# jimouris/draft-mouris-cfrg-mastic

Hardware: AMD Instinct MI355X
Metric: VIDPF report x prefix evals/sec at 1/2/4/8 GPUs; % of int-VALU peak (higher is better)
Workload: dtype u32

## Files before the change

draft-mouris-cfrg-mastic_amd/csrc/keccak.hpp:

```cpp
#pragma once
#include "common.hpp"

#define KECCAK_RATE 168
#define KECCAK_RATE_WORDS 42

struct KState {
    u32x2 a[25];
};

#define KR(x, y) KECCAK_ROTC[(x) + 5 * (y)]
static constexpr int KECCAK_ROTC[25] = {0,  1,  62, 28, 27, 36, 44, 6,  55, 20, 3,  10, 43,
                                        25, 39, 41, 45, 15, 21, 8,  18, 2,  61, 56, 14};

MH_D u32x2 chi1(u32x2 a, u32x2 b, u32x2 c) {
    return u32x2{(uint32_t)__builtin_amdgcn_bitop3_b32(a.lo, b.lo, c.lo, 0xD2),
                 (uint32_t)__builtin_amdgcn_bitop3_b32(a.hi, b.hi, c.hi, 0xD2)};
}

template <int U = 12, bool FUSE_D = true>
MH_D void keccak_p12(KState& s) {
    static constexpr uint32_t RCL[12] = {0x8000808bu, 0x0000008bu, 0x00008089u, 0x00008003u,
                                         0x00008002u, 0x00000080u, 0x0000800au, 0x8000000au,
                                         0x80008081u, 0x00008080u, 0x80000001u, 0x80008008u};
    static constexpr uint32_t RCH[12] = {0x00000000u, 0x80000000u, 0x80000000u, 0x80000000u,
                                         0x80000000u, 0x80000000u, 0x00000000u, 0x80000000u,
                                         0x80000000u, 0x80000000u, 0x00000000u, 0x80000000u};
    u32x2* A = s.a;
#pragma unroll U
    for (int round = 0; round < 12; round++) {
        u32x2 C[5], D[5];
#pragma unroll
        for (int x = 0; x < 5; x++) {
            u32x2 t = xor3_64(A[x], A[x + 5], A[x + 10]);
            C[x] = xor3_64(t, A[x + 15], A[x + 20]);
        }
        u32x2 B[25];
        if constexpr (FUSE_D) {
#pragma unroll
            for (int x = 0; x < 5; x++) D[x] = rotl64(C[(x + 1) % 5], 1);
#pragma unroll
            for (int x = 0; x < 5; x++)
#pragma unroll
                for (int y = 0; y < 5; y++)
                    B[y + 5 * ((2 * x + 3 * y) % 5)] = rotl64(xor3_64(A[x + 5 * y], C[(x + 4) % 5], D[x]), KR(x, y));
        } else {
#pragma unroll
            for (int x = 0; x < 5; x++) D[x] = xor64(C[(x + 4) % 5], rotl64(C[(x + 1) % 5], 1));
#pragma unroll
            for (int x = 0; x < 5; x++)
#pragma unroll
                for (int y = 0; y < 5; y++)
                    B[y + 5 * ((2 * x + 3 * y) % 5)] = rotl64(xor64(A[x + 5 * y], D[x]), KR(x, y));
        }
#pragma unroll
        for (int y = 0; y < 5; y++)
#pragma unroll
            for (int x = 0; x < 5; x++)
                A[x + 5 * y] = chi1(B[x + 5 * y], B[(x + 1) % 5 + 5 * y], B[(x + 2) % 5 + 5 * y]);
        A[0].lo ^= RCL[round];
        A[0].hi ^= RCH[round];
    }
}

struct KHalf {
    uint32_t a[25];
};

MH_D uint32_t pair_swap(uint32_t v) {
    return (uint32_t)__builtin_amdgcn_mov_dpp((int)v, 0xB1, 0xF, 0xF, false);
}

MH_D uint32_t pair_rotl(uint32_t v, int r) {
    if (r == 0) return v;
    const uint32_t p = pair_swap(v);
    return r < 32 ? __builtin_amdgcn_alignbit(v, p, 32 - r) : __builtin_amdgcn_alignbit(p, v, 64 - r);
}

template <int U = 12>
MH_D void keccak_p12_pair(KHalf& s, bool hi) {
    static constexpr uint32_t RCL[12] = {0x8000808bu, 0x0000008bu, 0x00008089u, 0x00008003u,
                                         0x00008002u, 0x00000080u, 0x0000800au, 0x8000000au,
                                         0x80008081u, 0x00008080u, 0x80000001u, 0x80008008u};
    static constexpr uint32_t RCH[12] = {0x00000000u, 0x80000000u, 0x80000000u, 0x80000000u,
                                         0x80000000u, 0x80000000u, 0x00000000u, 0x80000000u,
                                         0x80000000u, 0x80000000u, 0x00000000u, 0x80000000u};
    uint32_t* A = s.a;
#pragma unroll U
    for (int round = 0; round < 12; round++) {
        uint32_t C[5], D[5];
#pragma unroll
        for (int x = 0; x < 5; x++) C[x] = xor3_u32(xor3_u32(A[x], A[x + 5], A[x + 10]), A[x + 15], A[x + 20]);
#pragma unroll
        for (int x = 0; x < 5; x++) D[x] = pair_rotl(C[(x + 1) % 5], 1);
        uint32_t B[25];
#pragma unroll
        for (int x = 0; x < 5; x++)
#pragma unroll
            for (int y = 0; y < 5; y++)
                B[y + 5 * ((2 * x + 3 * y) % 5)] = pair_rotl(xor3_u32(A[x + 5 * y], C[(x + 4) % 5], D[x]), KR(x, y));
#pragma unroll
        for (int y = 0; y < 5; y++)
#pragma unroll
            for (int x = 0; x < 5; x++)
                A[x + 5 * y] = (uint32_t)__builtin_amdgcn_bitop3_b32(B[x + 5 * y], B[(x + 1) % 5 + 5 * y],
                                                                    B[(x + 2) % 5 + 5 * y], 0xD2);
        A[0] ^= hi ? RCH[round] : RCL[round];
    }
}

MH_D uint32_t kword(const KState& s, int j) {
    return (j & 1) ? s.a[j >> 1].hi : s.a[j >> 1].lo;
}
MH_D void kxor_word(KState& s, int j, uint32_t v) {
    if (j & 1) s.a[j >> 1].hi ^= v; else s.a[j >> 1].lo ^= v;
}

template <class Loader>
MH_D int sponge_absorb_words(KState& s, int f, int nbytes, Loader ld) {
    if (nbytes <= 0) return f;
    const int q = f >> 2;
    const int sh = f & 3;
    const int off = sh ? 1 : 0;
    const int amt = (32 - 8 * sh) & 31;
    const int nw = (nbytes + 3) >> 2;
    const int end = f + nbytes;
    for (int b = 0;; b++) {
        const int base = KECCAK_RATE_WORDS * b - q - off;
        uint32_t w[KECCAK_RATE_WORDS + 1];
#pragma unroll
        for (int j = 0; j < KECCAK_RATE_WORDS + 1; j++) {
            const int m = base + j;
            w[j] = ld(m < 0 ? 0 : (m >= nw ? nw - 1 : m));
        }
#pragma unroll
        for (int j = 0; j < KECCAK_RATE_WORDS + 1; j++) {
            const int m = base + j;
            w[j] = (m >= 0 && m < nw) ? w[j] : 0u;
        }
#pragma unroll
        for (int j = 0; j < KECCAK_RATE_WORDS; j++) kxor_word(s, j, __builtin_amdgcn_alignbit(w[j + 1], w[j], amt));
        if (end >= KECCAK_RATE * (b + 1)) {
            keccak_p12(s);
            if (end == KECCAK_RATE * (b + 1)) return 0;
        } else {
            return end - KECCAK_RATE * b;
        }
    }
}

MH_D void sponge_pad(KState& s, int f, uint32_t domain) {
    const int q = f >> 2;
    const uint32_t dw = domain << (8 * (f & 3));
// ... 58 lines not shown
```

draft-mouris-cfrg-mastic_amd/csrc/kernels.hpp:

```cpp
#pragma once
#include "aes.hpp"
#include "flp.hpp"
#include "keccak.hpp"

enum PfxId {
    PFX_EXT = 0,
    PFX_CONV,
    PFX_NODE,
    PFX_ONEHOT,
    PFX_PAYLOAD,
    PFX_EVAL,
    PFX_QUERY,
    PFX_PROOF_SHARE,
    PFX_JR_PART,
    PFX_JR_SEED,
    PFX_JR,
    PFX_PROVE_RAND,
    PFX_TREE,
    PFX_COUNT
};

struct PrefixState {
    KState st;
    int f;
// ... 533 lines not shown
        } else {
            const uint32_t* const sd2[2] = {cv, cv};
            const uint32_t cvv[2] = {c0, c1};
            uint32_t* const ov[2] = {o[0], o[1]};
            fixed_key_block_n<2>(TL, rkc, sd2, cvv, ov);
        }
        bool sus = false;
        const int e0 = EPB * b;
#pragma unroll
        for (int k = 0; k < 2 * EPB; k++) {
            const int e = e0 + k;
            const uint32_t top = EPB == 2 ? o[k >> 1][2 * (k & 1) + 1] : o[k][3];
            if (e < e_hi && (k < EPB || two)) sus |= top == ~0u;
        }
        if (__builtin_expect(__any(sus), 0) || b == force_slow_blk || b + 1 == force_slow_blk) break;
        __builtin_amdgcn_s_waitcnt(0x0F70);
#pragma unroll
        for (int k = 0; k < 2 * EPB; k++) {
            const int e = e0 + k;
            if (e < e_hi && (k < EPB || two)) {
                E x = F::from_words(&o[k / EPB][(k % EPB) * F::W32]);
                if (t) x = F::add(x, cwv[k]);
                pl_store<F>(out, row0 + e, S, r, x);
            }
        }
        e_fast = min(e_hi, e0 + 2 * EPB);
    }
    if (e_fast < e_hi) {
        typename EvalStream<F, false>::type st;
        st.init(cv);
        for (int e = 0; e < e_hi; e++) {
            asm volatile("" ::: "memory");
            const E x = st.next(TL, rkc);
            if (e >= e_fast) put(e, x);
        }
    }
}

#define EVAL_WAVES 16
#ifndef MASTIC_EMIT_WAIT
#define MASTIC_EMIT_WAIT 1
#endif
#ifndef MASTIC_CTR_GROUPS
#define MASTIC_CTR_GROUPS 1
#endif
#define EVAL_PROOF_WAVES 8
#ifndef EVAL_MIN_WAVES
#define EVAL_MIN_WAVES 5
#endif
#ifndef EVAL_FC_MIN_WAVES
#define EVAL_FC_MIN_WAVES 4
#endif
#define EVAL_VGPR_ATTR __attribute__((amdgpu_waves_per_eu(FC ? EVAL_FC_MIN_WAVES : EVAL_MIN_WAVES)))
#define EVAL_SYNC_WORDS 40
#define EVAL_LDS_BYTES (AES_PERM_LDS_WORDS * 4 + 2 * 64 * 11 * 16 + 4 * EVAL_SYNC_WORDS)
template <class F, bool GEN, bool FC, bool SPLIT = false>
__global__ __launch_bounds__(64 * EVAL_WAVES) EVAL_VGPR_ATTR
void k_eval_aes(McParams p, Planes pl, AesArgs a) {
    typedef typename F::E E;
    extern __shared__ uint4 eval_lds[];
    uint32_t* T = (uint32_t*)eval_lds;
    uint4* RKE = eval_lds + AES_PERM_LDS_WORDS / 4;
    uint4* RKC = RKE + 64 * 11;
    uint32_t* next_parent = (uint32_t*)(RKC + 64 * 11);
    uint32_t* next_proof = next_parent + 1;
    uint32_t* parent_done = next_parent + 8;
    if ((uint32_t)(uintptr_t)(const __attribute__((address_space(3))) uint4*)eval_lds != 0u) __builtin_trap();

    const int S = pl.stride;
    const int S_in = FC ? a.in_stride : S;
    const int lane = threadIdx.x & 63;
    const int wave = __builtin_amdgcn_readfirstlane(threadIdx.x >> 6);
    const int r = blockIdx.x * 64 + lane;
    const uint32_t lb = (uint32_t)r * 4u;
    {
        uint32_t* ke = (uint32_t*)RKE;
        uint32_t* kc = (uint32_t*)RKC;
        constexpr int KR = (44 + EVAL_WAVES - 1) / EVAL_WAVES;
        uint32_t xe[KR], xc[KR];
#pragma unroll
        for (int j = 0; j < KR; j++) {
            const int i = wave + j * EVAL_WAVES;
            if (i < 44) {
                xe[j] = pld(pl.rk_ext + (size_t)i * S, lb);
                xc[j] = pld(pl.rk_conv + (size_t)i * S, lb);
            }
        }
        aes_perm_fill(T, threadIdx.x, 64 * EVAL_WAVES);
#pragma unroll
        for (int j = 0; j < KR; j++) {
            const int i = wave + j * EVAL_WAVES;
            if (i < 44) {
                ke[lane * 44 + i] = aes_perm_key_word(i, xe[j]);
                kc[lane * 44 + i] = aes_perm_key_word(i, xc[j]);
            }
        }
    }
    if (threadIdx.x < EVAL_SYNC_WORDS) next_parent[threadIdx.x] = (SPLIT && threadIdx.x >= 8) ? ~0u : 0u;
    __syncthreads();
    const int aes_waves = a.aes_waves;
    if (wave >= aes_waves && a.pv_nodes > 0 && !(a.dbg_skip & 1)) {
        if (a.proof_prio == 1) __builtin_amdgcn_s_setprio(1);
        if (a.proof_prio == 2) __builtin_amdgcn_s_setprio(2);
        const int nbeg = (blockIdx.y * (EVAL_WAVES - aes_waves) + (wave - aes_waves)) * a.pv_npw;
        const int nend = min(nbeg + a.pv_npw, a.pv_nodes);
        const int pl_ = a.pv_level;
        uint32_t* ohg = a.pv_onehot + (size_t)blockIdx.x * a.oh_gstride;
        const uint32_t lt = (uint32_t)lane * 4u;
        uint32_t pcw[8];
#pragma unroll
        for (int j = 0; j < 8; j++) pcw[j] = pld(pl.cw_proof + ((size_t)pl_ * 8 + j) * S, lb);
        for (int node = nbeg; node < nend; node++) {
            uint32_t sd[4];
#pragma unroll
            for (int i = 0; i < 4; i++) sd[i] = pld(a.cs_in + ((size_t)node * 5 + i) * S_in, lb);
            const uint32_t t = pld(a.cs_in + ((size_t)node * 5 + 4) * S_in, lb);
            node_proof_one<FC>(a.np, a.np_f, p.bits, pl_, a.pv_path_bytes, sd, a.pv_child_path + node * 8, t, pcw,
                           [&](int j, uint32_t w) { pst(ohg + ((size_t)node * 8 + j) * a.bin_rstride, lt, w); });
        }
        if (a.proof_prio) __builtin_amdgcn_s_setprio(0);
    }
    const int wp0 = blockIdx.y * a.par_waves * a.ppw;
    const int wp1 = min(wp0 + a.par_waves * a.ppw, SPLIT ? a.n_parents * a.split : a.n_parents);
    const int pn_beg = 2 * wp0, pn_end = 2 * wp1;
    const bool fuse_ovl = FC && a.fuse_proofs == 1;
    auto parent_marked = [&](int q) -> bool {
        const uint32_t w = __hip_atomic_load(parent_done + (q >> 5), __ATOMIC_ACQUIRE, __HIP_MEMORY_SCOPE_WORKGROUP);
        return (__builtin_amdgcn_readfirstlane(w) >> (q & 31)) & 1u;
    };
    auto claim_node = [&]() -> int {
        uint32_t o = 0;
        if (lane == 0) o = atomicAdd(next_proof, 1u);
        return pn_beg + (int)__builtin_amdgcn_readfirstlane(o);
    };
    auto node_proof_at = [&](int node) {
        if (a.dbg_skip & 2) return;
        if (fuse_ovl)
            while (!parent_marked((node - pn_beg) >> 1)) __builtin_amdgcn_s_sleep(2);
        const int l = a.level;
        uint32_t* ohg = a.cur_onehot + (size_t)blockIdx.x * a.oh_gstride;
        const uint32_t lt = (uint32_t)lane * 4u;
        uint32_t pcw[8];
#pragma unroll
        for (int j = 0; j < 8; j++) pcw[j] = pld(pl.cw_proof + ((size_t)l * 8 + j) * S, lb);
        uint32_t sd[4];
#pragma unroll
        for (int i = 0; i < 4; i++) sd[i] = pld(a.cs_out + ((size_t)node * 5 + i) * S, lb);
        const uint32_t t = pld(a.cs_out + ((size_t)node * 5 + 4) * S, lb);
        node_proof_one<FC>(a.np, a.np_f, p.bits, l, a.cur_path_bytes, sd, a.cur_child_path + node * 8, t, pcw,
                       [&](int j, uint32_t w) { pst(ohg + ((size_t)node * 8 + j) * a.bin_rstride, lt, w); });
    };
    if (a.dbg_skip & 2) goto aes_done;
    if (fuse_ovl && wave >= aes_waves) goto aes_done;
    {
    if (a.aes_prio == 1) __builtin_amdgcn_s_setprio(1);
    if (a.aes_prio == 2) __builtin_amdgcn_s_setprio(2);
    const int l = a.level;
    const int vl = p.value_len;
    const int wl = vl * F::W32;
    const AesPerm TL{T, 4u * (uint32_t)(lane & 31), 128u + 4u * (uint32_t)(lane & 31)};
    const RkLds rke{RKE + lane * 11};
    const RkLds rkc{RKC + lane * 11};

    uint32_t scw[4];
#pragma unroll
    for (int i = 0; i < 4; i++) scw[i] = pld(pl.cw_seed + ((size_t)l * 4 + i) * S, lb);
    const uint32_t ccw = pld(pl.cw_ctrl + (size_t)l * S, lb);
    const uint32_t* wcw = pl.cw_w + (size_t)l * wl * S;

    const int K = SPLIT ? a.split : 1;
    constexpr int npass = SPLIT ? 2 : 1;
// ... 225 lines not shown
                if constexpr (EPB == 2)
                    sus = (o0[1] == ~0u) | (o1[1] == ~0u) | (two & ((o0[3] == ~0u) | (o1[3] == ~0u)));
                else
                    sus = (o0[3] == ~0u) | (o1[3] == ~0u);
                if (__builtin_expect(__any(sus), 0) || b == a.force_slow_blk) {
                    if (K > 1) {
                        if (lane == 0) atomicMin(split_first + (pi - pb), (uint32_t)e);
                        deferred = true;
                    }
                    break;
                }
#if MASTIC_EMIT_WAIT
                __builtin_amdgcn_s_waitcnt(0x0F70);
#endif
                emit(e, F::from_words(o0), F::from_words(o1), cwa, wpa);
                if constexpr (EPB == 2) {
                    if (two) emit(e + 1, F::from_words(o0 + 2), F::from_words(o1 + 2), cwb, wpb);
                }
                e_fast = e + 1 + (two ? 1 : 0);
            }
        }
        if (e_fast < e_hi && !deferred) {
            typename EvalStream<F, false>::type st0, st1;
            st0.init(cs0);
            st1.init(cs1);
            constexpr int G = EvalStream<F, false>::type::GROUP;
            for (int e0 = 0; e0 < e_hi; e0 += G) {
                asm volatile("" ::: "memory");
                st0.refill(st1, e_hi - e0, TL, rkc);
#pragma unroll
                for (int i = 0; i < G; i++) {
                    const int e = e0 + i;
                    if (e >= e_hi) break;
                    const E x0 = st0.next(TL, rkc);
                    const E x1 = st1.next(TL, rkc);
                    if (e >= e_fast) emit(e, x0, x1, load_cw(e), load_wp(e));
                }
            }
        }
        item = nxt;
    }
    }
    }
aes_done:
    if constexpr (FC) {
        if (a.fuse_proofs) {
            if (!fuse_ovl) __syncthreads();
#pragma unroll 1
            for (int node = claim_node(); node < pn_end; node = claim_node()) node_proof_at(node);
        }
    }
}

struct ProofArgs {
    int oh_gstride;
    int bin_rstride;
    int level;
    int n_nodes;
    int npw;
    int path_bytes;
    const uint32_t* child_path;
    const uint32_t* cs;
    uint32_t* onehot;
    const PrefixState* np;
    int f;
};

__global__ __launch_bounds__(256) void k_node_proof(McParams p, Planes pl, ProofArgs a) {
    const int S = pl.stride;
    const int lane = threadIdx.x & 63;
    const int wave = __builtin_amdgcn_readfirstlane(threadIdx.x >> 6);
    const int r = blockIdx.x * 64 + lane;
    const uint32_t lb = (uint32_t)r * 4u;
    const int nbeg = (blockIdx.y * 4 + wave) * a.npw;
    if (nbeg >= a.n_nodes) return;
    const int nend = min(nbeg + a.npw, a.n_nodes);
    const int l = a.level;
    uint32_t* ohg = a.onehot + (size_t)blockIdx.x * a.oh_gstride;
    const uint32_t lt = (uint32_t)lane * 4u;
    uint32_t pcw[8];
#pragma unroll
    for (int j = 0; j < 8; j++) pcw[j] = pld(pl.cw_proof + ((size_t)l * 8 + j) * S, lb);
    for (int node = nbeg; node < nend; node++) {
        uint32_t seed[4];
#pragma unroll
        for (int i = 0; i < 4; i++) seed[i] = pld(a.cs + ((size_t)node * 5 + i) * S, lb);
        const uint32_t t = pld(a.cs + ((size_t)node * 5 + 4) * S, lb);
        node_proof_one(a.np, a.f, p.bits, l, a.path_bytes, seed, a.child_path + node * 8, t, pcw,
                       [&](int j, uint32_t w) { pst(ohg + ((size_t)node * 8 + j) * a.bin_rstride, lt, w); });
    }
}

struct AbsorbArgs {
    const uint32_t* seg[2];
    int gstride[2];
    int rstride;
    int nbytes[2];
    int f[2];
    int prio;
    int dbg;
    int which0;
};
MH_D void absorb_setprio(int prio) {
    switch (prio) {
        case 0: break;
        case 1: __builtin_amdgcn_s_setprio(1); break;
// ... 27 lines not shown
    const int end = f + nb;
    auto load_block = [&](int b, uint32_t* w) {
        const int base = KECCAK_RATE_WORDS * b - q - off;
        if (base >= 0 && base + KECCAK_RATE_WORDS < nw) {
            const __amdgpu_buffer_rsrc_t rs = mh_rsrc(seg + (size_t)base * a.rstride);
            uint32_t so = 0;
#pragma unroll
            for (int j = 0; j < KECCAK_RATE_WORDS + 1; j++) {
                w[j] = pld_so(rs, lt, so);
                so += rowb;
                asm volatile("" : "+s"(so));
            }
        } else {
#pragma unroll
            for (int j = 0; j < KECCAK_RATE_WORDS + 1; j++) {
                const int m = base + j;
                const int mc = m < 0 ? 0 : (m >= nw ? nw - 1 : m);
                w[j] = pld(seg + (size_t)mc * a.rstride, lt);
            }
#pragma unroll
            for (int j = 0; j < KECCAK_RATE_WORDS + 1; j++) {
                const int m = base + j;
                w[j] = (m >= 0 && m < nw) ? w[j] : 0u;
            }
        }
    };
    uint32_t cur[KECCAK_RATE_WORDS + 1];
    load_block(0, cur);
    for (int b = 0;; b++) {
        const bool full = end >= KECCAK_RATE * (b + 1);
        const bool more = end > KECCAK_RATE * (b + 1);
#pragma unroll
        for (int j = 0; j < KECCAK_RATE_WORDS; j++) kxor_word(s, j, __builtin_amdgcn_alignbit(cur[j + 1], cur[j], amt));
        if (!full) break;
        asm volatile("" ::: "memory");
        if (more) load_block(b + 1, cur);
#ifdef MASTIC_EXPERIMENT_KNOBS
        if (a.dbg == 3)
            keccak_p12<2>(s);
        else
#endif
            keccak_p12(s);
        if (!more) break;
    }
#pragma unroll
    for (int i = 0; i < 25; i++) {
        pst(sp + (size_t)(2 * i) * S, lb, s.a[i].lo);
        pst(sp + (size_t)(2 * i + 1) * S, lb, s.a[i].hi);
    }
}

#ifndef ABSORB_MIN_WAVES
#define ABSORB_MIN_WAVES 5
#endif
__global__ __launch_bounds__(256) __attribute__((amdgpu_waves_per_eu(ABSORB_MIN_WAVES)))
void k_absorb_pair(Planes pl, AbsorbArgs a) {
    absorb_setprio(a.prio);
    const int h = threadIdx.x & 1;
    const int r = blockIdx.x * (int)(blockDim.x >> 1) + (int)(threadIdx.x >> 1);
    const int which = a.which0 + (int)blockIdx.y;
    if (r >= pl.stride) return;
    const int nb = a.nbytes[which];
    if (nb == 0) return;
    const int S = pl.stride;
    uint32_t* sp = which == 0 ? pl.sp_onehot : pl.sp_payload;
    const uint32_t* seg = a.seg[which] + (size_t)(r >> 6) * a.gstride[which];
    const uint32_t lbh = ((uint32_t)h * (uint32_t)S + (uint32_t)r) * 4u;
    const uint32_t lt = (uint32_t)(r & 63) * 4u;
    const uint32_t rowb = (uint32_t)a.rstride * 4u;
    const uint32_t lth = lt + (uint32_t)h * rowb;
    const uint32_t rowb2 = 2u * rowb;
    KHalf s;
#pragma unroll
    for (int i = 0; i < 25; i++) s.a[i] = pld(sp + (size_t)(2 * i) * S, lbh);
    const int f = a.f[which];
    const int q = f >> 2;
    const int sh = f & 3;
    const int off = sh ? 1 : 0;
    const int amt = (32 - 8 * sh) & 31;
    const int nw = (nb + 3) >> 2;
    const int end = f + nb;
    constexpr int NL = KECCAK_RATE_WORDS / 2 + 1;
    auto load_block = [&](int b, uint32_t* w) {
        const int base = KECCAK_RATE_WORDS * b - q - off;
        if (base >= 0 && base + KECCAK_RATE_WORDS + 1 < nw) {
            const __amdgpu_buffer_rsrc_t rs = mh_rsrc(seg + (size_t)base * a.rstride);
            uint32_t so = 0;
#pragma unroll
            for (int k = 0; k < NL; k++) {
                w[k] = pld_so(rs, lth, so);
                so += rowb2;
                asm volatile("" : "+s"(so));
            }
        } else {
#pragma unroll
            for (int k = 0; k < NL; k++) {
                const int m = base + 2 * k + h;
                const int mc = m < 0 ? 0 : (m >= nw ? nw - 1 : m);
                w[k] = pld(seg, (uint32_t)mc * rowb + lt);
            }
#pragma unroll
            for (int k = 0; k < NL; k++) {
                const int m = base + 2 * k + h;
                w[k] = (m >= 0 && m < nw) ? w[k] : 0u;
            }
        }
    };
    uint32_t cur[NL];
    if (a.dbg == 1 || a.dbg == 4) {
#pragma unroll
        for (int k = 0; k < NL; k++) cur[k] = lt + k;
    } else {
        load_block(0, cur);
    }
    for (int b = 0;; b++) {
        const bool full = end >= KECCAK_RATE * (b + 1);
        const bool more = end > KECCAK_RATE * (b + 1);
#pragma unroll
        for (int i = 0; i < 21; i++) {
            uint32_t nxt = 0u;
            if (sh) {
                const uint32_t x0 = pair_swap(cur[i]), x1 = pair_swap(cur[i + 1]);
                nxt = h ? x1 : x0;
            }
            s.a[i] ^= __builtin_amdgcn_alignbit(nxt, cur[i], amt);
        }
        if (!full) break;
        asm volatile("" ::: "memory");
        if (more && a.dbg != 1 && a.dbg != 4) load_block(b + 1, cur);
        if (a.dbg == 0 || a.dbg == 1) keccak_p12_pair(s, h != 0);
        else if (a.dbg == 4) __builtin_amdgcn_s_sleep(72);
        if (!more) break;
    }
#pragma unroll
    for (int i = 0; i < 25; i++) pst(sp + (size_t)(2 * i) * S, lbh, s.a[i]);
}

struct FinalArgs {
    int agg_id;
    int f_onehot;
    int f_payload;
};

template <class F>
__global__ __launch_bounds__(256) void k_finalize(McParams p, Planes pl, FinalArgs a, const PrefixState* pfx) {
    __shared__ uint32_t V[24 * 256];
    const int r = blockIdx.x * 256 + threadIdx.x;
    if (r >= pl.stride) return;
    const int S = pl.stride;
    uint32_t oh[8], pc[8];
    {
        KState s;
#pragma unroll
        for (int i = 0; i < 25; i++) s.a[i] = u32x2{pl.sp_onehot[(2 * i) * S + r], pl.sp_onehot[(2 * i + 1) * S + r]};
        sponge_pad(s, a.f_onehot, 0x01);
#pragma unroll
        for (int j = 0; j < 8; j++) oh[j] = kword(s, j);
#pragma unroll
        for (int i = 0; i < 25; i++) s.a[i] = u32x2{pl.sp_payload[(2 * i) * S + r], pl.sp_payload[(2 * i + 1) * S + r]};
        sponge_pad(s, a.f_payload, 0x01);
#pragma unroll
        for (int j = 0; j < 8; j++) pc[j] = kword(s, j);
    }
    typename F::E cnt = F::add(pl_load<F>(pl.rootsum, 0, S, r), F::from_u64((uint64_t)a.agg_id));
    const int t = threadIdx.x;
    for (int j = 0; j < 8; j++) V[j * 256 + t] = oh[j];
    for (int j = 0; j < F::W32; j++) V[(8 + j) * 256 + t] = F::word(cnt, j);
    for (int j = 0; j < 8; j++) V[(8 + F::W32 + j) * 256 + t] = pc[j];
    KState s;
    int f;
    load_prefix(pfx, PFX_EVAL, s, f);
    f = sponge_absorb_words(s, f, 64 + F::ENC, [&](int m) { return V[m * 256 + t]; });
    sponge_pad(s, f, 0x01);
#pragma unroll
    for (int j = 0; j < 8; j++) pl.eval_proof[j * S + r] = kword(s, j);
}

template <class F, class Put>
MH_D void squeeze_elems(KState& s, int count, Put put) {
    sponge_squeeze_vec<F::W32>(
        s, count, [&](const uint32_t* w) { return F::valid(F::from_words(w)); },
        [&](int e, const uint32_t* w) { put(e, F::from_words(w)); });
}
// ... 234 lines not shown
```

draft-mouris-cfrg-mastic_amd/csrc/mastic_hip.hip:

```cpp
#include "mastic_hip.h"

#include <dlfcn.h>
#include <rccl/rccl.h>

#include <algorithm>
#include <atomic>
#include <chrono>
#include <condition_variable>
#include <cstdarg>
#include <cstdio>
#include <cstring>
#include <map>
#include <memory>
#include <mutex>
#include <string>
#include <system_error>
#include <thread>
#include <type_traits>
#include <vector>

#include "comm_agree.hpp"
#include "host_tree.hpp"
#include "kernels.hpp"
#include "shard.hpp"
// ... 135 lines not shown
    int comm_timeout_ms = MASTIC_COMM_TIMEOUT_MS;
    DevBuf comm_local, comm_gather, comm_out;
    DevBuf comm_st;
    void* comm_st_host = nullptr;
    size_t comm_st_host_n = 0;
    void comm_release();
    PrefixState pfx_host[PFX_COUNT];
    std::string err;
    uint64_t budget = 0;
    DevBuf work;
    DevBuf pfx;
    DevBuf pfx_bytes, pfx_meta;
    DevBuf consts;
    DevBuf agg_valid, agg_out;
    DevBuf agg_part;
    DevBuf stage;
    int absorb_mode = 0;
    size_t absorb_single_min = 65536;
    int absorb_lds = 0;
    int n_cus = 256;
    int proof_waves = EVAL_PROOF_WAVES;
    int hit_proof_waves = 0;
    int proof_prio = 0;
    int aes_prio = 0;
    int dbg_skip = 0;
    int stride_pad = 64;
    size_t work_arena = (size_t)48 << 30;
    size_t work_arena_fc = (size_t)128 << 30;
    bool binder_tiled = true;
    int absorb_threads = 256;
    int absorb_prio = 3;
    int absorb_dbg = 0;
    int force_slow_blk = -1;
    int fail_allocs = 0;
    int sponge_delay_us = 0;
    int wall_khz = 100000;
    bool timing_nowait = false;
    bool serial_sponges = false;
    bool inject_alloc_failure() {
        if (fail_allocs <= 0) return false;
        fail_allocs--;
        return true;
    }
    bool idle() {
        return hipStreamSynchronize(stream) == hipSuccess && hipStreamSynchronize(stream2) == hipSuccess &&
               hipStreamSynchronize(stream3) == hipSuccess && hipStreamSynchronize(stream4) == hipSuccess;
    }
    int split_sponges = -1;
    bool fuse_last_miss = false;
    bool fuse_last_miss_fc = true;
    bool hit_absorb_main = true;
    bool fc_all = false;
    bool small_split = true;
    int fuse_proofs = 1;
    size_t chunk_max = 0;
    bool chunk_pipeline = true;
    int par_waves = 0;
    int pfx_f[PFX_COUNT] = {0};
    std::vector<uint8_t> pfx_key;
    std::map<std::vector<uint8_t>, Tree*> trees;
    Result res[2];
    bool frontier_cache = false;
    bool last_hit = false;
    LevelCache lc[2];
    DevBuf fc_spare;
    size_t spare_cap = 0;
    size_t spare_S = 0;
    std::vector<void*> graveyard;
    struct {
        bool valid = false;
        uint64_t rep_id = 0, rep_gen = 0;
        size_t n = 0;
        int stride = 0;
        const void* W = nullptr;
        std::vector<uint8_t> pfx_key;
    } rk;
    void* tree_stage = nullptr;
    size_t tree_stage_bytes = 0;
    hipEvent_t tree_ev = nullptr;
    void bury() {
        for (void* q : graveyard) (void)hipFree(q);
        graveyard.clear();
    }
    struct Timing {
        std::vector<hipEvent_t> ev;
        double t_eval = 0, t_proof = 0, t_absorb = 0, t_total = 0;
        int n_eval = 0, n_absorb = 0;
    } tm[2];
    int tcur = 0;
    ~mastic_ctx() {
        bury();
        for (auto& kv : trees) delete kv.second;
        for (auto& x : tm)
            for (auto e : x.ev) (void)hipEventDestroy(e);
        for (auto e : sync_ev) (void)hipEventDestroy(e);
        if (fold_ev) (void)hipEventDestroy(fold_ev);
        for (hipEvent_t e : comm_marks)
            if (e) (void)hipEventDestroy(e);
        if (comm) comm_release();
        if (comm_st_host) (void)hipHostFree(comm_st_host);
        if (tree_ev) (void)hipEventDestroy(tree_ev);
        if (tree_stage) (void)hipHostFree(tree_stage);
        if (stream) (void)hipStreamDestroy(stream);
        if (stream2) (void)hipStreamDestroy(stream2);
        if (stream3) (void)hipStreamDestroy(stream3);
        if (stream4) (void)hipStreamDestroy(stream4);
// ... 424 lines not shown
        const size_t max_words = std::max<size_t>((size_t)p.value_len * p.w32 * (l_hi - l_lo),
                                                  agg_id == 0 ? (size_t)p.proof_len * p.w32 : 0);
        const bool tiles = row_bytes >= 16384 && (((uintptr_t)pub | (uintptr_t)in_b | ps | is | nctrl) & 7) == 0 &&
                           (max_words + 63) / 64 < 65535;
        hipLaunchKernelGGL(k_unpack, dim3((n + 255) / 256), dim3(256), 0, c->stream, p, pl, agg_id,
                           rep->nonces.as<uint8_t>() + 16 * base, pub, in_b, l_lo, l_hi, tiles ? 1 : 0);
        if (tiles) {
            const int wlw_ = p.value_len * p.w32, nl = l_hi - l_lo;
            auto rows = [&](const uint8_t* src, size_t row_bytes, int nwords, uint32_t* dst) {
                if (nwords <= 0) return;
                hipLaunchKernelGGL(k_rows_to_planes, dim3((unsigned)((n + 63) / 64), (unsigned)((nwords + 63) / 64)),
                                   dim3(256), 0, c->stream, src, row_bytes, n, nwords, dst, stride);
            };
            const uint8_t* seg = pub + nctrl;
            rows(seg + 16 * (size_t)l_lo, ps, 4 * nl, pl.cw_seed + (size_t)4 * l_lo * stride);
            seg += 16 * (size_t)p.bits;
            rows(seg + (size_t)l_lo * p.value_len * p.enc, ps, wlw_ * nl, pl.cw_w + (size_t)wlw_ * l_lo * stride);
            seg += (size_t)p.bits * p.value_len * p.enc;
            rows(seg + 32 * (size_t)l_lo, ps, 8 * nl, pl.cw_proof + (size_t)8 * l_lo * stride);
            if (agg_id == 0) rows(in_b + 16, is, p.proof_len * p.w32, pl.lps);
        }
        HIPCHK(c, hipGetLastError());
    }
    const bool whole = base == 0 && (size_t)n == rep->n && W == c->work.p;
    const bool rk_ok = hit && whole && c->rk.valid && c->rk.rep_id == rep->id && c->rk.rep_gen == rep->generation() &&
                       c->rk.n == (size_t)n && c->rk.stride == stride && c->rk.W == (const void*)W &&
                       c->rk.pfx_key == c->pfx_key;
    if (!rk_ok) {
        hipLaunchKernelGGL(k_setup, dim3((stride + 255) / 256), dim3(256), 0, c->stream, pl, pfx, hit ? 0 : 1);
        c->rk.valid = whole;
        c->rk.rep_id = rep->id;
        c->rk.rep_gen = rep->generation();
        c->rk.n = (size_t)n;
        c->rk.stride = stride;
        c->rk.W = (const void*)W;
        c->rk.pfx_key = c->pfx_key;
    }
    HIPCHK(c, hipGetLastError());

    const int groups = (n + 63) / 64;
    const int wlw = p.value_len * p.w32;
    int f_oh = c->pfx_f[PFX_ONEHOT], f_pl = c->pfx_f[PFX_PAYLOAD];
    auto plane = [&](size_t off) { return W + off * (size_t)stride; };
    size_t sev = sev0;
    std::vector<hipEvent_t> abs_done(t->L + 1);
    const int oh_gstride = c->binder_tiled ? t->max_level_nodes * 8 * 64 : 64;
    const int pay_gstride = c->binder_tiled ? t->max_parents * wlw * 64 : 64;
    const int bin_rstride = c->binder_tiled ? 64 : stride;
    auto oh_buf = [&](int lv) -> uint32_t* { return plane(wl.onehot[lv % NSLOT]); };
    auto pay_buf = [&](int lv) -> uint32_t* { return plane(wl.payload[lv % NSLOT]); };
    auto oh_gs = [&](int) -> int { return oh_gstride; };
    auto pay_gs = [&](int) -> int { return pay_gstride; };
    const bool pair = c->absorb_mode == 2 || (c->absorb_mode == 0 && (size_t)n < c->absorb_single_min);
    auto launch_sponges = [&](int lv, int which0, int nwh, hipEvent_t ready, hipEvent_t e4, hipEvent_t e5,
                              hipStream_t as, hipEvent_t* done) -> int {
        AbsorbArgs ab;
        ab.which0 = which0;
        ab.seg[0] = oh_buf(lv);
        ab.gstride[0] = oh_gs(lv);
        ab.nbytes[0] = 2 * t->n_parents[lv] * 32;
        ab.f[0] = f_oh;
        ab.seg[1] = pay_buf(lv);
        ab.gstride[1] = pay_gs(lv);
        ab.rstride = bin_rstride;
        ab.nbytes[1] = lv > 0 ? t->n_parents[lv] * wlw * 4 : 0;
        ab.f[1] = f_pl;
        ab.prio = c->absorb_prio;
        ab.dbg = c->absorb_dbg;
        if (as != c->stream) HIPCHK(c, hipStreamWaitEvent(as, ready, 0));
        if (e4) HIPCHK(c, hipEventRecord(e4, as));
        if (c->dbg_skip & 4) {
        } else if (pair)
            hipLaunchKernelGGL(k_absorb_pair,
                               dim3((groups * 64 * 2 + c->absorb_threads - 1) / c->absorb_threads, (unsigned)nwh),
                               dim3(c->absorb_threads), c->absorb_lds, as, pl, ab);
        else
            hipLaunchKernelGGL(k_absorb, dim3((groups * 64 + 255) / 256, (unsigned)nwh), dim3(256), c->absorb_lds, as,
                               pl, ab);
        if (e5) HIPCHK(c, hipEventRecord(e5, as));
        HIPCHK(c, hipGetLastError());
        *done = get_sync_event(c, sev++);
        HIPCHK(c, hipEventRecord(*done, as));
        if (c->serial_sponges && as != c->stream) HIPCHK(c, hipStreamWaitEvent(c->stream, *done, 0));
        if (which0 == 0) f_oh = (f_oh + ab.nbytes[0]) % KECCAK_RATE;
        if (which0 + nwh > 1) f_pl = (f_pl + ab.nbytes[1]) % KECCAK_RATE;
        return 0;
    };
    std::vector<hipEvent_t> pl_done(t->L + 1, nullptr);
    auto launch_absorb = [&](int lv, hipEvent_t ready, hipEvent_t e4, hipEvent_t e5, hipStream_t as) -> int {
        return launch_sponges(lv, 0, 2, ready, e4, e5, as, &abs_done[lv]);
    };
    const bool split_on = c->split_sponges < 0 ? p.field == 128 : c->split_sponges > 0;
    const bool split = split_on && !hit && tail == c->stream && ss == c->stream2;
    auto from_cache = [&](uint32_t* dst, const uint32_t* src, size_t planes) -> int {
        HIPCHK(c, hipMemcpy2DAsync(dst, (size_t)stride * 4, src + base, lc->S * 4, (size_t)n * 4, planes,
                                   hipMemcpyDeviceToDevice, c->stream));
        return 0;
    };
    auto to_cache = [&](uint32_t* dst, const uint32_t* src, size_t planes) -> int {
        HIPCHK(c, hipMemcpy2DAsync(dst + base, lc->S * 4, src, (size_t)stride * 4, (size_t)n * 4, planes,
                                   hipMemcpyDeviceToDevice, tail));
        return 0;
    };
    if (hit && !direct) {
        if (from_cache(pl.sp_onehot, lc->sp.as<uint32_t>(), 50)) return -1;
        if (from_cache(pl.sp_payload, lc->sp.as<uint32_t>() + (size_t)50 * lc->S, 50)) return -1;
// ... 33 lines not shown
        const int n_items = np_ * a.split;
        a.ppw = choose_eval_ppw(n_items, groups, par_waves, c->n_cus);
        if (a.split > 1) a.ppw = (n_items + par_waves - 1) / par_waves;
        a.parent_node = t->d_parent + t->poff[l];
        a.child_exp = t->d_exp + t->off[l];
        a.child_pfx = t->d_pfx + t->off[l];
        a.cs_in = hit ? cin + base : plane(wl.cs[(l + 1) & 1]);
        a.cs_out = plane(wl.cs[l & 1]);
        a.fr_w_in = plane(wl.fr_w[(l + 1) & 1]);
        a.in_stride = hit ? (int)lc->S : stride;
        a.fr_w_out = plane(wl.fr_w[l & 1]);
        a.payload = pay_buf(l);
        a.out = R.out.as<uint32_t>() + base;
        a.out_stride = (int)R.stride;
        a.force_slow_blk = c->force_slow_blk;
        a.cache_out = (lc && l == t->L) ? cout + base : nullptr;
        a.cache_stride = lc ? (int)lc->S : 0;
        a.wp_buf = plane(wl.fr_w[(l + 1) & 1]);
        a.recompute_wp = hit ? 1 : 0;
        const bool fuse = fuse_last && l == t->L;
        a.fuse_proofs = fuse ? (c->fuse_proofs == 3 ? 3 : 1) : 0;
        a.cur_path_bytes = (l + 1 + 7) / 8;
        a.cur_child_path = t->d_path + t->off[l] * 8;
        a.cur_onehot = oh_buf(l);
        a.aes_waves = EVAL_WAVES - c->proof_waves;
        if (fuse && a.fuse_proofs == 1)
            a.aes_waves = EVAL_WAVES - (hit ? hit_proof_waves(p, c) : miss_proof_waves(p, c, t->n_parents[l - 1 < 0 ? 0 : l - 1],
                                                                                      np_, l > 0));
        a.par_waves = par_waves;
        a.proof_prio = c->proof_prio;
        a.aes_prio = c->aes_prio;
        a.dbg_skip = c->dbg_skip;
        const int gy = (n_items + a.par_waves * a.ppw - 1) / (a.par_waves * a.ppw);
        a.pv_level = l - 1;
        a.pv_nodes = (l > 0 && !hit) ? 2 * t->n_parents[l - 1] : 0;
        const int pw = EVAL_WAVES - a.aes_waves;
        a.pv_npw = (a.pv_nodes + gy * pw - 1) / (gy * pw);
        a.pv_path_bytes = (l + 7) / 8;
        a.pv_child_path = l > 0 ? t->d_path + t->off[l - 1] * 8 : nullptr;
        a.pv_onehot = l > 0 ? oh_buf(l - 1) : nullptr;
        a.oh_gstride = l > 0 ? oh_gs(l - 1) : oh_gstride;
        a.pay_gstride = pay_gs(l);
        a.bin_rstride = bin_rstride;
        a.np = (const PrefixState*)c->pfx.p + PFX_NODE;
        a.np_f = c->pfx_f[PFX_NODE];
        dim3 grid(groups, gy);
        hipEvent_t e0 = get_event(c, evi++), e1 = get_event(c, evi++);
        hipEvent_t e2 = get_event(c, evi++), e3 = get_event(c, evi++);
        hipEvent_t e4 = get_event(c, evi++), e5 = get_event(c, evi++);
        HIPCHK(c, hipEventRecord(e0, c->stream));
        if ((lc && (hit || l == t->L || c->fc_all)) || fuse)
            hipLaunchKernelGGL((k_eval_aes<F, true, true>), grid, dim3(64 * EVAL_WAVES), EVAL_LDS_BYTES, c->stream,
                               p, pl, a);
        else if (a.split > 1 && l == 0)
            hipLaunchKernelGGL((k_eval_aes<F, true, false, true>), grid, dim3(64 * EVAL_WAVES), EVAL_LDS_BYTES,
                               c->stream, p, pl, a);
        else if (a.split > 1)
            hipLaunchKernelGGL((k_eval_aes<F, false, false, true>), grid, dim3(64 * EVAL_WAVES), EVAL_LDS_BYTES,
                               c->stream, p, pl, a);
        else if (l == 0 || l == t->L)
            hipLaunchKernelGGL((k_eval_aes<F, true, false>), grid, dim3(64 * EVAL_WAVES), EVAL_LDS_BYTES, c->stream,
                               p, pl, a);
        else
            hipLaunchKernelGGL((k_eval_aes<F, false, false>), grid, dim3(64 * EVAL_WAVES), EVAL_LDS_BYTES, c->stream,
                               p, pl, a);
        HIPCHK(c, hipEventRecord(e1, c->stream));
        HIPCHK(c, hipGetLastError());
        HIPCHK(c, hipEventRecord(e2, c->stream));
        HIPCHK(c, hipEventRecord(e3, c->stream));
        hipEvent_t aes_done = get_sync_event(c, sev++);
        HIPCHK(c, hipEventRecord(aes_done, c->stream));
        if (split && l > 0) {
            if (launch_sponges(l, 1, 1, aes_done, e4, e5, c->stream3, &pl_done[l])) return -1;
            if (launch_sponges(l - 1, 0, 1, aes_done, nullptr, nullptr, ss, &abs_done[l - 1])) return -1;
        } else if (l > 0 && !hit) {
            if (launch_absorb(l - 1, aes_done, e4, e5, ss)) return -1;
        } else {
            if (c->sponge_delay_us > 0) {
                const unsigned long long ticks =
                    (unsigned long long)c->sponge_delay_us * (unsigned long long)c->wall_khz / 1000;
                c->sponge_delay_us = 0;
                hipLaunchKernelGGL(k_spin, dim3(1), dim3(64), 0, ss, ticks);
                HIPCHK(c, hipGetLastError());
            }
            HIPCHK(c, hipEventRecord(e4, ss));
            HIPCHK(c, hipEventRecord(e5, ss));
        }
    }
    if (fuse_last) {
        const int l = t->L;
        hipEvent_t e0 = get_event(c, evi++), e1 = get_event(c, evi++);
        hipEvent_t e2 = get_event(c, evi++), e3 = get_event(c, evi++);
        hipEvent_t e4 = get_event(c, evi++), e5 = get_event(c, evi++);
        HIPCHK(c, hipEventRecord(e0, c->stream));
        HIPCHK(c, hipEventRecord(e1, c->stream));
        HIPCHK(c, hipEventRecord(e2, c->stream));
        HIPCHK(c, hipEventRecord(e3, c->stream));
        hipEvent_t np_done = get_sync_event(c, sev++);
        HIPCHK(c, hipEventRecord(np_done, c->stream));
        if (split ? launch_sponges(l, 0, 1, np_done, e4, e5, last_as, &abs_done[l])
                  : launch_absorb(l, np_done, e4, e5, last_as))
            return -1;
    } else {
        const int l = t->L;
        const int nn = 2 * t->n_parents[l];
        ProofArgs pa;
// ... 1276 lines not shown
        if (hipDeviceGetAttribute(&khz, hipDeviceAttributeWallClockRate, up->device) == hipSuccess && khz > 0)
            c->wall_khz = khz;
    }
#ifdef MASTIC_EXPERIMENT_KNOBS
    {
        const char* e = getenv("MASTIC_ABSORB_SINGLE");
        if (e) c->absorb_mode = e[0] == '1' ? 1 : (e[0] == '2' ? 2 : 0);
        const char* esm = getenv("MASTIC_ABSORB_SINGLE_MIN");
        if (esm) c->absorb_single_min = (size_t)std::max(0, atoi(esm));
        const char* l = getenv("MASTIC_ABSORB_LDS_KB");
        c->absorb_lds = l ? std::max(0, std::min(160, atoi(l))) * 1024 : 0;
        const char* pw = getenv("MASTIC_PROOF_WAVES");
        if (pw) c->proof_waves = std::max(1, std::min(15, atoi(pw)));
        const char* spd = getenv("MASTIC_STRIDE_PAD");
        if (spd) c->stride_pad = std::max(0, std::min(1 << 20, atoi(spd))) / 64 * 64;
        const char* wa = getenv("MASTIC_WORK_ARENA_GB");
        if (wa) c->work_arena = c->work_arena_fc = (size_t)std::max(0, atoi(wa)) << 30;
        const char* bt = getenv("MASTIC_BINDER_TILED");
        if (bt) c->binder_tiled = bt[0] != '0';
        const char* at = getenv("MASTIC_ABSORB_THREADS");
        if (at) c->absorb_threads = std::max(64, std::min(256, atoi(at))) / 64 * 64;
        const char* ap = getenv("MASTIC_ABSORB_PRIO");
        if (ap) c->absorb_prio = std::max(0, std::min(3, atoi(ap)));
        const char* adb = getenv("MASTIC_ABSORB_DBG");
        if (adb) c->absorb_dbg = atoi(adb);
        const char* dsk = getenv("MASTIC_DBG_SKIP");
        if (dsk) c->dbg_skip = atoi(dsk);
        const char* xp = getenv("MASTIC_AES_PRIO");
        if (xp) c->aes_prio = std::max(0, std::min(2, atoi(xp)));
        const char* pp = getenv("MASTIC_PROOF_PRIO");
        if (pp) c->proof_prio = std::max(0, std::min(2, atoi(pp)));
        const char* pw2 = getenv("MASTIC_PAR_WAVES");
        if (pw2) c->par_waves = std::max(1, std::min(EVAL_WAVES, atoi(pw2)));
        const char* cp = getenv("MASTIC_CHUNK_PIPELINE");
        if (cp) c->chunk_pipeline = cp[0] != '0';
        const char* hpw = getenv("MASTIC_HIT_PROOF_WAVES");
        if (hpw) c->hit_proof_waves = std::max(0, std::min(15, atoi(hpw)));
        const char* fp = getenv("MASTIC_FUSE_PROOFS");
        if (fp) c->fuse_proofs = std::max(0, std::min(3, atoi(fp)));
        const char* fa = getenv("MASTIC_FC_ALL");
        if (fa) c->fc_all = fa[0] == '1';
        const char* cr = getenv("MASTIC_CHUNK_REPORTS");
        if (cr) c->chunk_max = (size_t)std::max(0, atoi(cr));
        const char* spl = getenv("MASTIC_SPLIT_SPONGES");
        if (spl) c->split_sponges = spl[0] == '1' ? 1 : 0;
        const char* flm = getenv("MASTIC_FUSE_LAST_MISS");
        if (flm) c->fuse_last_miss = flm[0] == '1';
        const char* flf = getenv("MASTIC_FUSE_LAST_MISS_FC");
        if (flf) c->fuse_last_miss_fc = flf[0] != '0';
        const char* ham = getenv("MASTIC_HIT_ABSORB_MAIN");
        if (ham) c->hit_absorb_main = ham[0] != '0';
        const char* ssp = getenv("MASTIC_SMALL_SPLIT");
        if (ssp) c->small_split = ssp[0] != '0';
        const char* tnw = getenv("MASTIC_DBG_TIMING_NOWAIT");
        if (tnw) c->timing_nowait = tnw[0] == '1';
        const char* ssr = getenv("MASTIC_SERIAL_SPONGES");
        if (ssr) c->serial_sponges = ssr[0] == '1';
    }
#endif
    if (hipFuncSetAttribute((const void*)k_eval_aes<F64, false, false>, hipFuncAttributeMaxDynamicSharedMemorySize,
                            EVAL_LDS_BYTES) != hipSuccess ||
        hipFuncSetAttribute((const void*)k_eval_aes<F128, false, false>, hipFuncAttributeMaxDynamicSharedMemorySize,
                            EVAL_LDS_BYTES) != hipSuccess ||
        hipFuncSetAttribute((const void*)k_eval_aes<F64, true, false>, hipFuncAttributeMaxDynamicSharedMemorySize,
                            EVAL_LDS_BYTES) != hipSuccess ||
        hipFuncSetAttribute((const void*)k_eval_aes<F128, true, false>, hipFuncAttributeMaxDynamicSharedMemorySize,
                            EVAL_LDS_BYTES) != hipSuccess ||
        hipFuncSetAttribute((const void*)k_eval_aes<F64, true, true>, hipFuncAttributeMaxDynamicSharedMemorySize,
                            EVAL_LDS_BYTES) != hipSuccess ||
        hipFuncSetAttribute((const void*)k_eval_aes<F128, true, true>, hipFuncAttributeMaxDynamicSharedMemorySize,
                            EVAL_LDS_BYTES) != hipSuccess ||
        hipFuncSetAttribute((const void*)k_eval_aes<F64, true, false, true>,
                            hipFuncAttributeMaxDynamicSharedMemorySize, EVAL_LDS_BYTES) != hipSuccess ||
        hipFuncSetAttribute((const void*)k_eval_aes<F64, false, false, true>,
                            hipFuncAttributeMaxDynamicSharedMemorySize, EVAL_LDS_BYTES) != hipSuccess ||
        hipFuncSetAttribute((const void*)k_eval_aes<F128, true, false, true>,
                            hipFuncAttributeMaxDynamicSharedMemorySize, EVAL_LDS_BYTES) != hipSuccess ||
        hipFuncSetAttribute((const void*)k_eval_aes<F128, false, false, true>,
                            hipFuncAttributeMaxDynamicSharedMemorySize, EVAL_LDS_BYTES) != hipSuccess ||
        hipFuncSetAttribute((const void*)k_absorb_pair, hipFuncAttributeMaxDynamicSharedMemorySize, 160 * 1024) !=
            hipSuccess ||
        hipFuncSetAttribute((const void*)k_absorb, hipFuncAttributeMaxDynamicSharedMemorySize, 160 * 1024) !=
            hipSuccess) {
        delete c;
        return MASTIC_EHIP;
    }
    int prio_lo = 0, prio_hi = 0;
    (void)hipDeviceGetStreamPriorityRange(&prio_lo, &prio_hi);
    if (hipStreamCreateWithFlags(&c->stream, hipStreamNonBlocking) != hipSuccess ||
        hipStreamCreateWithPriority(&c->stream2, hipStreamNonBlocking, prio_hi) != hipSuccess ||
        hipStreamCreateWithPriority(&c->stream3, hipStreamNonBlocking, prio_hi) != hipSuccess ||
        hipStreamCreateWithFlags(&c->stream4, hipStreamNonBlocking) != hipSuccess) {
        delete c;
        return MASTIC_EHIP;
    }
    *out = c;
    return 0;
}

extern "C" void mastic_ctx_destroy(mastic_ctx* c) {
    DeviceScope ds_(c);
    if (!c) return;
    (void)hipStreamSynchronize(c->stream);
    (void)hipStreamSynchronize(c->stream2);
    (void)hipStreamSynchronize(c->stream3);
    (void)hipStreamSynchronize(c->stream4);
    delete c;
}

extern "C" const char* mastic_last_error(const mastic_ctx* c) { return c ? c->err.c_str() : "null ctx"; }

extern "C" int mastic_set_frontier_cache(mastic_ctx* c, int on, int* last_hit) {
    DeviceScope ds_(c);
    if (!c) return MASTIC_EINVAL;
    if (on >= 0) {
        c->frontier_cache = on != 0;
        if (!on) {
            for (auto& x : c->lc) {
                for (DevBuf* b : {&x.sp, &x.rootsum, &x.nd}) {
                    if (b->p && b->own) c->graveyard.push_back(b->p);
                    b->p = nullptr;
                    b->bytes = 0;
                }
                x.release();
            }
            if (c->fc_spare.p && c->fc_spare.own) c->graveyard.push_back(c->fc_spare.p);
            c->fc_spare.p = nullptr;
            c->fc_spare.bytes = 0;
            c->spare_cap = 0;
            c->spare_S = 0;
        }
    }
// ... 55 lines not shown
```

Measured before the change: 138.2 million.

## Add register-capped wide eval kernel variant and cheaper pair-swap selection in absorb

```diff
diff --git a/draft-mouris-cfrg-mastic_amd/csrc/keccak.hpp b/draft-mouris-cfrg-mastic_amd/csrc/keccak.hpp
--- a/draft-mouris-cfrg-mastic_amd/csrc/keccak.hpp
+++ b/draft-mouris-cfrg-mastic_amd/csrc/keccak.hpp
@@ -66,8 +66,10 @@
     uint32_t a[25];
 };
 
+template <bool SWZ = false>
 MH_D uint32_t pair_swap(uint32_t v) {
-    return (uint32_t)__builtin_amdgcn_mov_dpp((int)v, 0xB1, 0xF, 0xF, false);
+    if constexpr (SWZ) return (uint32_t)__builtin_amdgcn_ds_swizzle((int)v, 0x80B1);
+    else return (uint32_t)__builtin_amdgcn_mov_dpp((int)v, 0xB1, 0xF, 0xF, false);
 }
 
 MH_D uint32_t pair_rotl(uint32_t v, int r) {
@@ -76,7 +78,7 @@
     return r < 32 ? __builtin_amdgcn_alignbit(v, p, 32 - r) : __builtin_amdgcn_alignbit(p, v, 64 - r);
 }
 
-template <int U = 12>
+template <int U = 12, bool SWZ = false>
 MH_D void keccak_p12_pair(KHalf& s, bool hi) {
     static constexpr uint32_t RCL[12] = {0x8000808bu, 0x0000008bu, 0x00008089u, 0x00008003u,
                                          0x00008002u, 0x00000080u, 0x0000800au, 0x8000000au,
@@ -90,14 +92,38 @@
         uint32_t C[5], D[5];
 #pragma unroll
         for (int x = 0; x < 5; x++) C[x] = xor3_u32(xor3_u32(A[x], A[x + 5], A[x + 10]), A[x + 15], A[x + 20]);
-#pragma unroll
-        for (int x = 0; x < 5; x++) D[x] = pair_rotl(C[(x + 1) % 5], 1);
         uint32_t B[25];
-#pragma unroll
-        for (int x = 0; x < 5; x++)
-#pragma unroll
-            for (int y = 0; y < 5; y++)
-                B[y + 5 * ((2 * x + 3 * y) % 5)] = pair_rotl(xor3_u32(A[x + 5 * y], C[(x + 4) % 5], D[x]), KR(x, y));
+        if constexpr (SWZ) {
+            uint32_t P[5];
+#pragma unroll
+            for (int x = 0; x < 5; x++) P[x] = pair_swap<true>(C[(x + 1) % 5]);
+#pragma unroll
+            for (int x = 0; x < 5; x++) D[x] = __builtin_amdgcn_alignbit(C[(x + 1) % 5], P[x], 31);
+            uint32_t T[25], Q[25];
+#pragma unroll
+            for (int i = 0; i < 25; i++) T[i] = xor3_u32(A[i], C[(i % 5 + 4) % 5], D[i % 5]);
+            B[0] = T[0];
+#pragma unroll
+            for (int st = 0; st < 2; st++) {
+#pragma unroll
+                for (int i = 1 + 12 * st; i < 13 + 12 * st; i++) Q[i] = pair_swap<true>(T[i]);
+#pragma unroll
+                for (int i = 1 + 12 * st; i < 13 + 12 * st; i++) {
+                    const int x = i % 5, y = i / 5, r = KR(x, y);
+                    B[y + 5 * ((2 * x + 3 * y) % 5)] = r < 32 ? __builtin_amdgcn_alignbit(T[i], Q[i], 32 - r)
+                                                              : __builtin_amdgcn_alignbit(Q[i], T[i], 64 - r);
+                }
+            }
+        } else {
+#pragma unroll
+            for (int x = 0; x < 5; x++) D[x] = pair_rotl(C[(x + 1) % 5], 1);
+#pragma unroll
+            for (int x = 0; x < 5; x++)
+#pragma unroll
+                for (int y = 0; y < 5; y++)
+                    B[y + 5 * ((2 * x + 3 * y) % 5)] =
+                        pair_rotl(xor3_u32(A[x + 5 * y], C[(x + 4) % 5], D[x]), KR(x, y));
+        }
 #pragma unroll
         for (int y = 0; y < 5; y++)
 #pragma unroll
diff --git a/draft-mouris-cfrg-mastic_amd/csrc/kernels.hpp b/draft-mouris-cfrg-mastic_amd/csrc/kernels.hpp
--- a/draft-mouris-cfrg-mastic_amd/csrc/kernels.hpp
+++ b/draft-mouris-cfrg-mastic_amd/csrc/kernels.hpp
@@ -609,11 +609,11 @@
 #define EVAL_FC_MIN_WAVES 4
 #endif
 #define EVAL_VGPR_ATTR __attribute__((amdgpu_waves_per_eu(FC ? EVAL_FC_MIN_WAVES : EVAL_MIN_WAVES)))
+#define EVAL_WIDE_ATTR __attribute__((amdgpu_waves_per_eu(4), amdgpu_num_vgpr(52)))
 #define EVAL_SYNC_WORDS 40
 #define EVAL_LDS_BYTES (AES_PERM_LDS_WORDS * 4 + 2 * 64 * 11 * 16 + 4 * EVAL_SYNC_WORDS)
-template <class F, bool GEN, bool FC, bool SPLIT = false>
-__global__ __launch_bounds__(64 * EVAL_WAVES) EVAL_VGPR_ATTR
-void k_eval_aes(McParams p, Planes pl, AesArgs a) {
+template <class F, bool GEN, bool FC, bool SPLIT, bool WIDE>
+MH_D void eval_aes_body(const McParams& p, const Planes& pl, const AesArgs& a) {
     typedef typename F::E E;
     extern __shared__ uint4 eval_lds[];
     uint32_t* T = (uint32_t*)eval_lds;
@@ -665,15 +665,29 @@
         uint32_t* ohg = a.pv_onehot + (size_t)blockIdx.x * a.oh_gstride;
         const uint32_t lt = (uint32_t)lane * 4u;
         uint32_t pcw[8];
-#pragma unroll
-        for (int j = 0; j < 8; j++) pcw[j] = pld(pl.cw_proof + ((size_t)pl_ * 8 + j) * S, lb);
+        if constexpr (!WIDE) {
+#pragma unroll
+            for (int j = 0; j < 8; j++) pcw[j] = pld(pl.cw_proof + ((size_t)pl_ * 8 + j) * S, lb);
+        }
         for (int node = nbeg; node < nend; node++) {
             uint32_t sd[4];
 #pragma unroll
             for (int i = 0; i < 4; i++) sd[i] = pld(a.cs_in + ((size_t)node * 5 + i) * S_in, lb);
-            const uint32_t t = pld(a.cs_in + ((size_t)node * 5 + 4) * S_in, lb);
-            node_proof_one<FC>(a.np, a.np_f, p.bits, pl_, a.pv_path_bytes, sd, a.pv_child_path + node * 8, t, pcw,
-                           [&](int j, uint32_t w) { pst(ohg + ((size_t)node * 8 + j) * a.bin_rstride, lt, w); });
+            if constexpr (WIDE) {
+                uint32_t w8[8];
+                node_proof_one<true>(a.np, a.np_f, p.bits, pl_, a.pv_path_bytes, sd, a.pv_child_path + node * 8, 0u, pcw,
+                                     [&](int j, uint32_t w) { w8[j] = w; });
+                const uint32_t t = pld(a.cs_in + ((size_t)node * 5 + 4) * S_in, lb);
+#pragma unroll
+                for (int j = 0; j < 8; j++) pcw[j] = pld(pl.cw_proof + ((size_t)pl_ * 8 + j) * S, lb);
+#pragma unroll
+                for (int j = 0; j < 8; j++)
+                    pst(ohg + ((size_t)node * 8 + j) * a.bin_rstride, lt, w8[j] ^ (t ? pcw[j] : 0u));
+            } else {
+                const uint32_t t = pld(a.cs_in + ((size_t)node * 5 + 4) * S_in, lb);
+                node_proof_one<FC>(a.np, a.np_f, p.bits, pl_, a.pv_path_bytes, sd, a.pv_child_path + node * 8, t, pcw,
+                                   [&](int j, uint32_t w) { pst(ohg + ((size_t)node * 8 + j) * a.bin_rstride, lt, w); });
+            }
         }
         if (a.proof_prio) __builtin_amdgcn_s_setprio(0);
     }
@@ -1005,6 +1019,17 @@
     }
 }
 
+template <class F, bool GEN, bool FC, bool SPLIT = false>
+__global__ __launch_bounds__(64 * EVAL_WAVES) EVAL_VGPR_ATTR
+void k_eval_aes(McParams p, Planes pl, AesArgs a) {
+    eval_aes_body<F, GEN, FC, SPLIT, false>(p, pl, a);
+}
+template <class F, bool GEN, bool SPLIT = false>
+__global__ __launch_bounds__(64 * EVAL_WAVES) EVAL_WIDE_ATTR
+void k_eval_aes_wide(McParams p, Planes pl, AesArgs a) {
+    eval_aes_body<F, GEN, false, SPLIT, true>(p, pl, a);
+}
+
 struct ProofArgs {
     int oh_gstride;
     int bin_rstride;
@@ -1138,6 +1163,9 @@
 
 #ifndef ABSORB_MIN_WAVES
 #define ABSORB_MIN_WAVES 5
+#endif
+#ifndef MASTIC_PAIR_SWZ
+#define MASTIC_PAIR_SWZ 0
 #endif
 __global__ __launch_bounds__(256) __attribute__((amdgpu_waves_per_eu(ABSORB_MIN_WAVES)))
 void k_absorb_pair(Planes pl, AbsorbArgs a) {
@@ -1193,6 +1221,7 @@
         }
     };
     uint32_t cur[NL];
+    const uint32_t hmask = 0u - (uint32_t)h;
     if (a.dbg == 1 || a.dbg == 4) {
 #pragma unroll
         for (int k = 0; k < NL; k++) cur[k] = lt + k;
@@ -1205,16 +1234,13 @@
 #pragma unroll
         for (int i = 0; i < 21; i++) {
             uint32_t nxt = 0u;
-            if (sh) {
-                const uint32_t x0 = pair_swap(cur[i]), x1 = pair_swap(cur[i + 1]);
-                nxt = h ? x1 : x0;
-            }
+            if (sh) nxt = pair_swap<MASTIC_PAIR_SWZ != 0>((uint32_t)__builtin_amdgcn_bitop3_b32(hmask, cur[i], cur[i + 1], 0xCA));
             s.a[i] ^= __builtin_amdgcn_alignbit(nxt, cur[i], amt);
         }
         if (!full) break;
         asm volatile("" ::: "memory");
         if (more && a.dbg != 1 && a.dbg != 4) load_block(b + 1, cur);
-        if (a.dbg == 0 || a.dbg == 1) keccak_p12_pair(s, h != 0);
+        if (a.dbg == 0 || a.dbg == 1) keccak_p12_pair<12, MASTIC_PAIR_SWZ != 0>(s, h != 0);
         else if (a.dbg == 4) __builtin_amdgcn_s_sleep(72);
         if (!more) break;
     }
diff --git a/draft-mouris-cfrg-mastic_amd/csrc/mastic_hip.hip b/draft-mouris-cfrg-mastic_amd/csrc/mastic_hip.hip
--- a/draft-mouris-cfrg-mastic_amd/csrc/mastic_hip.hip
+++ b/draft-mouris-cfrg-mastic_amd/csrc/mastic_hip.hip
@@ -211,6 +211,7 @@
     bool hit_absorb_main = true;
     bool fc_all = false;
     bool small_split = true;
+    bool eval_wide = true;
     int fuse_proofs = 1;
     size_t chunk_max = 0;
     bool chunk_pipeline = true;
@@ -741,6 +742,7 @@
     auto oh_gs = [&](int) -> int { return oh_gstride; };
     auto pay_gs = [&](int) -> int { return pay_gstride; };
     const bool pair = c->absorb_mode == 2 || (c->absorb_mode == 0 && (size_t)n < c->absorb_single_min);
+    const bool wide = pair && c->eval_wide;
     auto launch_sponges = [&](int lv, int which0, int nwh, hipEvent_t ready, hipEvent_t e4, hipEvent_t e5,
                               hipStream_t as, hipEvent_t* done) -> int {
         AbsorbArgs ab;
@@ -880,6 +882,18 @@
         if ((lc && (hit || l == t->L || c->fc_all)) || fuse)
             hipLaunchKernelGGL((k_eval_aes<F, true, true>), grid, dim3(64 * EVAL_WAVES), EVAL_LDS_BYTES, c->stream,
                                p, pl, a);
+        else if (wide && a.split > 1 && l == 0)
+            hipLaunchKernelGGL((k_eval_aes_wide<F, true, true>), grid, dim3(64 * EVAL_WAVES), EVAL_LDS_BYTES,
+                               c->stream, p, pl, a);
+        else if (wide && a.split > 1)
+            hipLaunchKernelGGL((k_eval_aes_wide<F, false, true>), grid, dim3(64 * EVAL_WAVES), EVAL_LDS_BYTES,
+                               c->stream, p, pl, a);
+        else if (wide && (l == 0 || l == t->L))
+            hipLaunchKernelGGL((k_eval_aes_wide<F, true>), grid, dim3(64 * EVAL_WAVES), EVAL_LDS_BYTES, c->stream,
+                               p, pl, a);
+        else if (wide)
+            hipLaunchKernelGGL((k_eval_aes_wide<F, false>), grid, dim3(64 * EVAL_WAVES), EVAL_LDS_BYTES, c->stream,
+                               p, pl, a);
         else if (a.split > 1 && l == 0)
             hipLaunchKernelGGL((k_eval_aes<F, true, false, true>), grid, dim3(64 * EVAL_WAVES), EVAL_LDS_BYTES,
                                c->stream, p, pl, a);
@@ -2262,6 +2276,8 @@
         if (ham) c->hit_absorb_main = ham[0] != '0';
         const char* ssp = getenv("MASTIC_SMALL_SPLIT");
         if (ssp) c->small_split = ssp[0] != '0';
+        const char* evw = getenv("MASTIC_EVAL_WIDE");
+        if (evw) c->eval_wide = evw[0] != '0';
         const char* tnw = getenv("MASTIC_DBG_TIMING_NOWAIT");
         if (tnw) c->timing_nowait = tnw[0] == '1';
         const char* ssr = getenv("MASTIC_SERIAL_SPONGES");
@@ -2288,6 +2304,22 @@
                             hipFuncAttributeMaxDynamicSharedMemorySize, EVAL_LDS_BYTES) != hipSuccess ||
         hipFuncSetAttribute((const void*)k_eval_aes<F128, false, false, true>,
                             hipFuncAttributeMaxDynamicSharedMemorySize, EVAL_LDS_BYTES) != hipSuccess ||
+        hipFuncSetAttribute((const void*)k_eval_aes_wide<F64, false>, hipFuncAttributeMaxDynamicSharedMemorySize,
+                            EVAL_LDS_BYTES) != hipSuccess ||
+        hipFuncSetAttribute((const void*)k_eval_aes_wide<F128, false>, hipFuncAttributeMaxDynamicSharedMemorySize,
+                            EVAL_LDS_BYTES) != hipSuccess ||
+        hipFuncSetAttribute((const void*)k_eval_aes_wide<F64, true>, hipFuncAttributeMaxDynamicSharedMemorySize,
+                            EVAL_LDS_BYTES) != hipSuccess ||
+        hipFuncSetAttribute((const void*)k_eval_aes_wide<F128, true>, hipFuncAttributeMaxDynamicSharedMemorySize,
+                            EVAL_LDS_BYTES) != hipSuccess ||
+        hipFuncSetAttribute((const void*)k_eval_aes_wide<F64, true, true>,
+                            hipFuncAttributeMaxDynamicSharedMemorySize, EVAL_LDS_BYTES) != hipSuccess ||
+        hipFuncSetAttribute((const void*)k_eval_aes_wide<F64, false, true>,
+                            hipFuncAttributeMaxDynamicSharedMemorySize, EVAL_LDS_BYTES) != hipSuccess ||
+        hipFuncSetAttribute((const void*)k_eval_aes_wide<F128, true, true>,
+                            hipFuncAttributeMaxDynamicSharedMemorySize, EVAL_LDS_BYTES) != hipSuccess ||
+        hipFuncSetAttribute((const void*)k_eval_aes_wide<F128, false, true>,
+                            hipFuncAttributeMaxDynamicSharedMemorySize, EVAL_LDS_BYTES) != hipSuccess ||
         hipFuncSetAttribute((const void*)k_absorb_pair, hipFuncAttributeMaxDynamicSharedMemorySize, 160 * 1024) !=
             hipSuccess ||
         hipFuncSetAttribute((const void*)k_absorb, hipFuncAttributeMaxDynamicSharedMemorySize, 160 * 1024) !=
```

After: 140.0 million, median of 6. 1.01x the previous value.
